# microsoft/GenerativeImage2Text

Measured on AMD Instinct MI355X. Metric: captions/sec whole-node (GIT_BASE 224px bs=64/GPU greedy len=20), higher is better.
Workload: dtype f16; 1 GPU; GIT_BASE 224px bs=64/GPU greedy max_len=20 frames=1; global_batch=64, parallelism=dp1, decode_steps_per_caption=19, seq_len_returned=20, hip_graph=True, contexts_in_flight=4, layernorm_folded=True, library=libgitmi_f16.so, encoder_chains=2, schedule=mixed

## Files before the change

generativeimage2text_amd/csrc/kernels_gemm10.hip:

```cpp
#include "gitmi_common.h"
#include "launchers.h"
#include <type_traits>

namespace gitmi {

namespace {

constexpr int BN = 256, BK = 64;
constexpr int HALF_BYTES = 128 * BK * 2;
constexpr int BUF_BYTES = 4 * HALF_BYTES;
constexpr int LDS_BYTES = 2 * BUF_BYTES;
constexpr int SLOT_A0 = 0, SLOT_A1 = HALF_BYTES, SLOT_B0 = 2 * HALF_BYTES, SLOT_B1 = 3 * HALF_BYTES;

typedef __attribute__((address_space(3))) void lds_void_t;

#define P8_BARRIER()                           \
    do {                                       \
        __builtin_amdgcn_sched_barrier(0);     \
        __builtin_amdgcn_s_barrier();          \
        asm volatile("" ::: "memory");         \
        __builtin_amdgcn_sched_barrier(0);     \
    } while (0)

__device__ __forceinline__ float add_unfused(float a, float b) {
// ... 25 lines not shown
#define P8_LDS_BARRIER()                                   \
    do {                                                   \
        asm volatile("s_waitcnt lgkmcnt(0)" ::: "memory"); \
        __builtin_amdgcn_s_barrier();                      \
        asm volatile("" ::: "memory");                     \
    } while (0)

template <typename T> __device__ __forceinline__ uint32_t pack2o(float lo, float hi) {
    if constexpr (std::is_same<T, f16_t>::value) return pack2h(lo, hi);
    else return pack2bf(lo, hi);
}
template <typename T> __device__ __forceinline__ void unpack2o(uint32_t u, float& lo, float& hi) {
    if constexpr (std::is_same<T, f16_t>::value) unpack2h(u, lo, hi);
    else unpack2op(u, lo, hi);
}

template <int N> __device__ __forceinline__ void wait_vm() {
    if constexpr (N == 8) asm volatile("s_waitcnt vmcnt(8)" ::: "memory");
    else if constexpr (N == 4) asm volatile("s_waitcnt vmcnt(4)" ::: "memory");
    else if constexpr (N == 2) asm volatile("s_waitcnt vmcnt(2)" ::: "memory");
    else if constexpr (N == 0) asm volatile("s_waitcnt vmcnt(0)" ::: "memory");
}

template <typename TOut, int ACT, int DBG = 0, int MH = 128, int EPI = 1, int MH1 = MH, int LNF = 0>
__global__ __launch_bounds__(512) void gemm_p8_kernel(GemmArgs g) {
    static_assert(LNF == 0 || sizeof(TOut) == 2, "LayerNorm folding: 16-bit outputs only");
    static_assert(MH % 32 == 0 && MH1 % 32 == 0 && MH1 <= MH && MH <= 128, "half tiles: multiples of 32 rows, second <= first");
    constexpr int BM = MH + MH1, MI = MH / 32, MI1 = MH1 / 32;
    __shared__ __attribute__((aligned(16))) unsigned char smem[LDS_BYTES];

    const int tid = threadIdx.x;
    const int lane = tid & 63;
    const int wave = __builtin_amdgcn_readfirstlane(tid >> 6);
    const int grp = wave >> 2, wc = wave & 3;
    const int l15 = lane & 15, lg = lane >> 4;
    uint64_t ts[8];
    auto stamp = [&](int i) {
        if constexpr ((DBG & 16) != 0) {
            __builtin_amdgcn_sched_barrier(0);
            ts[2 * i] = __builtin_amdgcn_s_memtime();
            ts[2 * i + 1] = __builtin_amdgcn_s_memrealtime();
            __builtin_amdgcn_sched_barrier(0);
        }
    };
    auto stamps_out = [&]() {
        if constexpr ((DBG & 16) != 0) {
            if (tid == 0) {
                uint64_t* o = reinterpret_cast<uint64_t*>(const_cast<float*>(g.res)) + (size_t)blockIdx.x * 8;
#pragma unroll
                for (int i = 0; i < 8; ++i) o[i] = ts[i];
            }
        }
// ... 97 lines not shown
        __builtin_amdgcn_sched_barrier(0);
        read_a(sb, H0);
        if constexpr (MODE <= 1) { issue(1, 1, t + 1); wait_vm<8>(); } else { wait_vm<2>(); }
        P8_BARRIER();
        mma(acc[0][0], wf0, H0);
        P8_BARRIER();
        read_w(sb, 1, wf1);
        if constexpr (MODE <= 1) { issue(0, 1, t + 1); wait_vm<8>(); } else { wait_vm<0>(); }
        P8_BARRIER();
        mma(acc[0][1], wf1, H0);
        P8_BARRIER();
        read_a(sb, H1);
        if constexpr (MODE == 0) { issue(0, 0, t + 2); wait_vm<8>(); }
        P8_BARRIER();
        mma(acc[1][1], wf1, H1);
        P8_BARRIER();
        if constexpr (MODE == 0) { issue(1, 0, t + 2); wait_vm<8>(); }
        else if constexpr (MODE == 1) { wait_vm<4>(); }
        P8_BARRIER();
        mma(acc[1][0], wf0, H1);
        P8_BARRIER();
    };

    float lmean[2][MI], lrstd[2][MI];
    unsigned char* const ln_lds = smem + BUF_BYTES + SLOT_A1;
    if constexpr (LNF == 1) {
        const int r = lane >> 1, qm = r >> 4, l = r & 15;
        const int MHq = qm ? MH1 : MH, MIq = qm ? MI1 : MI;
        const int ii = wc < MIq ? wc : MIq - 1;
        const int m = m0 + qm * MH + grp * (MHq / 2) + ii * 16 + l;
        const int mc = m < g.M ? m : g.M - 1;
        const char* src = reinterpret_cast<const char*>(g.ln_part) + (size_t)mc * 32 + (lane & 1) * 16;
        __builtin_amdgcn_global_load_lds((const void*)src, (lds_void_t*)(ln_lds + wave * 1024), 16, 0, 0);
    }
    auto ln_rows = [&]() {
        if constexpr (LNF == 1) {
#pragma unroll
            for (int qm = 0; qm < 2; ++qm) {
                const int MIq = qm ? MI1 : MI;
                const int ii = lg < MIq ? lg : MIq - 1;
                const unsigned char* pr = ln_lds + (grp * 4 + ii) * 1024 + (qm * 16 + l15) * 32;
                const f32x4_t p0 = *reinterpret_cast<const f32x4_t*>(pr);
                const f32x4_t p1 = *reinterpret_cast<const f32x4_t*>(pr + 16);
                const float sx = (p0[0] + p0[2]) + (p1[0] + p1[2]);
                const float sq = (p0[1] + p0[3]) + (p1[1] + p1[3]);
                const float mean = sx * g.ln_inv_d;
                const float rstd = rsqrtf(fmaxf(sq * g.ln_inv_d - mean * mean, 0.f) + g.ln_eps);
#pragma unroll
                for (int i = 0; i < MIq; ++i) {
                    lmean[qm][i] = __shfl(mean, i * 16 + l15, 64);
                    lrstd[qm][i] = __shfl(rstd, i * 16 + l15, 64);
                    asm volatile("" : "+v"(lmean[qm][i]), "+v"(lrstd[qm][i]));
                }
            }
            __builtin_amdgcn_sched_barrier(0);
        }
    };
    const int nk = g.K / BK;
    issue(0, 0, 0); issue(1, 0, 0); issue(1, 1, 0); issue(0, 1, 0); issue(0, 0, 1); issue(1, 0, 1);
    wait_vm<8>();
    P8_BARRIER();
    ln_rows();
#pragma unroll
    for (int a = 0; a < 2; ++a)
#pragma unroll
        for (int b = 0; b < 2; ++b)
#pragma unroll
            for (int j = 0; j < 2; ++j)
#pragma unroll
                for (int i = 0; i < MI; ++i) acc[a][b][j][i] = f32x4_t{0.f, 0.f, 0.f, 0.f};
    if (grp == 1) P8_BARRIER();
    stamp(1);
    for (int t = 0; t < nk - 2; ++t) ktile(std::integral_constant<int, 0>{}, t);
    ktile(std::integral_constant<int, 1>{}, nk - 2);
    ktile(std::integral_constant<int, 2>{}, nk - 1);
    if (grp == 0) P8_BARRIER();
// ... 19 lines not shown
#pragma unroll
                    for (int i = 0; i < MI; ++i) sum += acc[a][b][j][i][0] + acc[a][b][j][i][1] + acc[a][b][j][i][2] + acc[a][b][j][i][3];
        if (sum == 12345.678f) C[0] = (TOut)0;
        stamp(3);
        stamps_out();
        return;
    }
    f32x4_t bias4[2][2];
#pragma unroll
    for (int qn = 0; qn < 2; ++qn)
#pragma unroll
        for (int j = 0; j < 2; ++j)
            bias4[qn][j] = g.bias ? *reinterpret_cast<const f32x4_t*>(g.bias + n0 + qn * 128 + wc * 32 + j * 16 + lg * 4)
                                  : f32x4_t{0.f, 0.f, 0.f, 0.f};

    f32x4_t cs4[2][2];
    if constexpr (LNF == 1) {
#pragma unroll
        for (int qn = 0; qn < 2; ++qn)
#pragma unroll
            for (int j = 0; j < 2; ++j)
                cs4[qn][j] = *reinterpret_cast<const f32x4_t*>(g.ln_colsum + n0 + qn * 128 + wc * 32 + j * 16 + lg * 4);
    }
    auto ln_apply = [&](float a, int qm, int qn, int j, int i, int r) -> float {
        if constexpr (LNF == 1) return lrstd[qm][i] * fmaf(-lmean[qm][i], cs4[qn][j][r], a);
        else return a;
    };

    if constexpr (sizeof(TOut) == 4 && EPI == 1) {
        float* Cf = reinterpret_cast<float*>(g.C);
        const float* R = g.res;
        const int col0 = n0 + wc * 32 + lg * 4;
        const bool has_res = R != nullptr && !(DBG & 1);
#pragma unroll
        for (int qm = 0; qm < 2; ++qm) {
            const int MIq = qm ? MI1 : MI, MHq = qm ? MH1 : MH;
            f32x4_t rr[MI][2][2];
            if (has_res) {
#pragma unroll
                for (int i = 0; i < MIq; ++i) {
                    const int m = m0 + qm * MH + grp * (MHq / 2) + i * 16 + l15;
                    const int mc = m < g.M ? m : g.M - 1;
                    const float* rp = R + (size_t)mc * g.ldr + col0;
#pragma unroll
                    for (int qn = 0; qn < 2; ++qn)
#pragma unroll
                        for (int j = 0; j < 2; ++j)
                            rr[i][qn][j] = *reinterpret_cast<const f32x4_t*>(rp + qn * 128 + j * 16);
// ... 9 lines not shown
#pragma unroll
                    for (int j = 0; j < 2; ++j) {
                        f32x4_t v;
#pragma unroll
                        for (int r = 0; r < 4; ++r) v[r] = apply_act_t<ACT>(acc[qm][qn][j][i][r] + bias4[qn][j][r]);
                        if (has_res) {
#pragma unroll
                            for (int r = 0; r < 4; ++r) v[r] = add_unfused(v[r], rr[i][qn][j][r]);
                        }
                        if (ok) *reinterpret_cast<f32x4_t*>(cp + qn * 128 + j * 16) = v;
                    }
            }
        }
        return;
    }

    float rgm[8], rbt[8];
    if constexpr (LNF == 2) {
        if (g.res_part) {
            ld8(g.res_gamma + n0 + (tid & 31) * 8, rgm);
            ld8(g.res_beta + n0 + (tid & 31) * 8, rbt);
        }
    }
#pragma unroll
    for (int qm = 0; qm < 2; ++qm)
#pragma unroll
        for (int s = 0; s < 2 / NQN; ++s) {
            const int MIq = qm ? MI1 : MI, MHq = qm ? MH1 : MH;
#pragma unroll
            for (int u = 0; u < NQN; ++u) {
                const int qn = s * NQN + u;
#pragma unroll
                for (int j = 0; j < 2; ++j) {
                    const int nl = u * 128 + wc * 32 + j * 16 + lg * 4;
#pragma unroll
                    for (int i = 0; i < MIq; ++i) {
                        float v[4];
#pragma unroll
                        for (int r = 0; r < 4; ++r) v[r] = apply_act_t<ACT>(ln_apply(acc[qm][qn][j][i][r], qm, qn, j, i, r) + bias4[qn][j][r]);
                        TOut* p = ep + (grp * (MHq / 2) + i * 16 + l15) * EPS + nl;
                        if constexpr (sizeof(TOut) == 4) {
                            *reinterpret_cast<f32x4_t*>(p) = f32x4_t{v[0], v[1], v[2], v[3]};
                        } else {
                            uint2 t2;
                            t2.x = pack2o<TOut>(v[0], v[1]);
                            t2.y = pack2o<TOut>(v[2], v[3]);
                            *reinterpret_cast<uint2*>(p) = t2;
                        }
                    }
                }
            }
            P8_LDS_BARRIER();
#pragma unroll 4
            for (int q = 0; q < MHq * CPR / 512; ++q) {
                const int chunk = tid + q * 512;
                const int row = chunk / CPR, cc = chunk % CPR;
                const int m = m0 + qm * MH + row;
                const int n = n0 + s * WCOL + cc * EPC;
                if (m < g.M && !(DBG & 1)) {
                    if constexpr (sizeof(TOut) == 4) {
                        f32x4_t v = *reinterpret_cast<const f32x4_t*>(ep + row * EPS + cc * EPC);
                        if (g.res && !(DBG & 16)) {
// ... 69 lines not shown
                            q2 = __builtin_elementwise_fma(x, x, q2);
                        }
                        float sx = s2[0] + s2[1], sq = q2[0] + q2[1];
                        half_wave_sum2_hi(sx, sq);
                        if (ok && cc == 16 && !(DBG & 1)) g.part_out[(size_t)m * 4 + tile_n] = float2{sx, sq};
                    }
                    if (ok && !(DBG & 1)) {
                        TOut* cp = C + (size_t)m * g.ldc + n;
                        asm volatile("global_store_dwordx4 %0, %1, off sc1\n\ts_nop 1" ::"v"(cp), "v"(v) : "memory");
                    }
                }
            }
            P8_LDS_BARRIER();
        }
    if constexpr ((DBG & 16) != 0) {
        asm volatile("s_waitcnt vmcnt(0)" ::: "memory");
        stamp(3);
        stamps_out();
    }
}

}

template <typename TOut, int MH, int EPI = 1, int MH1 = MH, int LNF = 0>
static void launch_p8_t(const GemmArgs& g, hipStream_t s) {
    if constexpr (LNF == 2) {
        hipLaunchKernelGGL((gemm_p8_kernel<TOut, GITMI_ACT_NONE, 0, MH, EPI, MH1, LNF>), dim3(g.nwg), dim3(512), 0, s, g);
        return;
    } else {
    if (g.dbg && LNF == 0) {
        if constexpr (MH == 128 && MH1 == 128) {
            switch (g.dbg) {
                case 1: hipLaunchKernelGGL((gemm_p8_kernel<TOut, 0, 1>), dim3(g.nwg), dim3(512), 0, s, g); return;
                case 2: hipLaunchKernelGGL((gemm_p8_kernel<TOut, 0, 2>), dim3(g.nwg), dim3(512), 0, s, g); return;
                case 6: hipLaunchKernelGGL((gemm_p8_kernel<TOut, 0, 6>), dim3(g.nwg), dim3(512), 0, s, g); return;
                case 10: hipLaunchKernelGGL((gemm_p8_kernel<TOut, 0, 10>), dim3(g.nwg), dim3(512), 0, s, g); return;
#ifdef GITMI_PROBE
                case 16: hipLaunchKernelGGL((gemm_p8_kernel<TOut, 0, 16>), dim3(g.nwg), dim3(512), 0, s, g); return;
                case 17: hipLaunchKernelGGL((gemm_p8_kernel<TOut, 0, 17>), dim3(g.nwg), dim3(512), 0, s, g); return;
                case 18: hipLaunchKernelGGL((gemm_p8_kernel<TOut, 0, 18>), dim3(g.nwg), dim3(512), 0, s, g); return;
                case 22: hipLaunchKernelGGL((gemm_p8_kernel<TOut, 0, 22>), dim3(g.nwg), dim3(512), 0, s, g); return;
                case 26: hipLaunchKernelGGL((gemm_p8_kernel<TOut, 0, 26>), dim3(g.nwg), dim3(512), 0, s, g); return;
#endif
                default: break;
            }
        }
    }
    switch (g.act) {
        case GITMI_ACT_QUICKGELU:
            hipLaunchKernelGGL((gemm_p8_kernel<TOut, GITMI_ACT_QUICKGELU, 0, MH, EPI, MH1, LNF>), dim3(g.nwg), dim3(512), 0, s, g); break;
        case GITMI_ACT_GELU_ERF:
            hipLaunchKernelGGL((gemm_p8_kernel<TOut, GITMI_ACT_GELU_ERF, 0, MH, EPI, MH1, LNF>), dim3(g.nwg), dim3(512), 0, s, g); break;
        default:
            hipLaunchKernelGGL((gemm_p8_kernel<TOut, GITMI_ACT_NONE, 0, MH, EPI, MH1, LNF>), dim3(g.nwg), dim3(512), 0, s, g); break;
    }
    }
}

bool gemm_p8_supports(const GemmArgs& g) {
    return g.K % BK == 0 && g.K >= 2 * BK && g.N % BN == 0 &&
           (double)g.M * g.lda * 2.0 < 4.0e9 && (double)g.N * g.K * 2.0 < 4.0e9;
}

static int p8_xcd_count(const GemmArgs& g, int bm, int ng, int* max_nn_out) {
    const int tiles_m = (g.M + bm - 1) / bm, tiles_n = g.N / BN, mg = 8 / ng;
    int max_cnt = 0, max_nn = 0;
    for (int x = 0; x < 8; ++x) {
        const int gn = x % ng, gm = x / ng;
        const int nn = (gn + 1) * tiles_n / ng - gn * tiles_n / ng;
        const int tg = tiles_m * nn;
        const int cnt = (gm + 1) * tg / mg - gm * tg / mg;
        max_cnt = cnt > max_cnt ? cnt : max_cnt;
        max_nn = nn > max_nn ? nn : max_nn;
    }
    if (max_nn_out) *max_nn_out = max_nn;
    return max_cnt;
}
static int p8_plan(const GemmArgs& g, int bm, int* ng_out, int* max_cnt_out) {
    const int tiles_n = g.N / BN;
    int best_ng = 1, best_rounds = 1 << 30, best_cnt = 0, best_panels = 1 << 30;
    for (int ng = 1; ng <= 8 && ng <= tiles_n; ng *= 2) {
        int max_nn = 0;
        const int max_cnt = p8_xcd_count(g, bm, ng, &max_nn);
        const int rounds = (max_cnt + 31) / 32;
        const int panels = (32 + max_nn - 1) / max_nn + (max_nn < 32 ? max_nn : 32);
        if (rounds < best_rounds || (rounds == best_rounds && panels < best_panels)) {
            best_ng = ng; best_rounds = rounds; best_cnt = max_cnt; best_panels = panels;
        }
    }
    if (ng_out) *ng_out = best_ng;
    if (max_cnt_out) *max_cnt_out = best_cnt;
    return best_rounds;
}

int gemm_p8_cost(const GemmArgs& g, int bm) {
    const int rounds = p8_plan(g, bm, nullptr, nullptr);
    const int ktile = 1450 * (90 + 166 * bm / 256) / 256;
    return rounds * (1450 + (g.K / BK) * ktile + 4700 * bm / 256);
}

template <int MH, int MH1>
static void launch_p8_height(const GemmArgs& g, bool out_f32, bool staged, hipStream_t s) {
#ifdef GITMI_OPS_F16
    if (g.ln_part) { launch_p8_t<bf16_t, MH, 1, MH1, 1>(g, s); return; }
    if (g.part_out || g.res_part) { launch_p8_t<f16_t, MH, 1, MH1, 2>(g, s); return; }
#endif
    if (g.out_f16) launch_p8_t<f16_t, MH, 1, MH1>(g, s);
    else if (!out_f32) launch_p8_t<bf16_t, MH, 1, MH1>(g, s);
    else if (staged) launch_p8_t<float, MH, 0, MH1>(g, s);
    else launch_p8_t<float, MH, 1, MH1>(g, s);
}

hipError_t launch_gemm_p8(GemmArgs g, bool out_f32, hipStream_t s) {
    if (g.ln_part || g.part_out || g.res_part) {
#ifndef GITMI_OPS_F16
        return hipErrorInvalidValue;
#endif
        if (g.ln_part && (out_f32 || g.out_f16 || g.res || !g.ln_colsum || g.ln_nparts < 1 || g.part_out || g.res_part)) return hipErrorInvalidValue;
        if ((g.part_out || g.res_part) && (!g.out_f16 || out_f32 || g.act != 0 || g.N > 1024)) return hipErrorInvalidValue;
        if (g.res_part && (!g.res || !g.res_gamma || !g.res_beta || g.res_nparts < 1)) return hipErrorInvalidValue;
    }
    static const int heights[5] = {256, 224, 192, 160, 128};
    int bm = 256;
    if (!g.shared) {
        int best = gemm_p8_cost(g, 256);
        for (int h = 1; h < 5; ++h) {
            const int c = gemm_p8_cost(g, heights[h]);
            if (c < best) { best = c; bm = heights[h]; }
        }
    }
    if (g.dbg & 64) bm = 192;
    if (g.dbg & 128) bm = 256;
    if (g.dbg & 16384) bm = 160;
    if (g.dbg & 32768) bm = 224;
    if (g.dbg & 65536) bm = 128;
    g.dbg &= ~(64 | 128 | 16384 | 32768 | 65536);
    g.tiles_n = g.N / BN;
    int max_cnt = 0;
    p8_plan(g, bm, &g.ng, &max_cnt);
    if (g.dbg & (1024 | 2048 | 4096 | 8192)) {
        const int ng = (g.dbg & 1024) ? 1 : (g.dbg & 2048) ? 2 : (g.dbg & 4096) ? 4 : 8;
        g.dbg &= ~(1024 | 2048 | 4096 | 8192);
        if (ng <= g.tiles_n) { g.ng = ng; max_cnt = p8_xcd_count(g, bm, ng, nullptr); }
    }
    g.nwg = 8 * max_cnt;
    const bool staged = (g.dbg & 256) != 0;
    g.dbg &= ~256;
    switch (bm) {
        case 224: launch_p8_height<128, 96>(g, out_f32, staged, s); break;
        case 192: launch_p8_height<96, 96>(g, out_f32, staged, s); break;
        case 160: launch_p8_height<96, 64>(g, out_f32, staged, s); break;
        case 128: launch_p8_height<64, 64>(g, out_f32, staged, s); break;
        default: launch_p8_height<128, 128>(g, out_f32, staged, s); break;
    }
    return hipGetLastError();
}

}
```

generativeimage2text_amd/engine.py:

```python
from __future__ import annotations

import ctypes as C
import os
from typing import Dict, List, Mapping, Optional, Sequence, Tuple

import torch

_HERE = os.path.dirname(os.path.abspath(__file__))
LIB_PATH = os.path.join(_HERE, "libgitmi.so")
LIB_PATH_F16 = os.path.join(_HERE, "libgitmi_f16.so")
LIB_PATH_EXP = os.path.join(_HERE, "libgitmi_exp.so")

PREC_BF16, PREC_F32 = 0, 1
DTYPE_F32, DTYPE_BF16, DTYPE_F16 = 0, 1, 2
DTYPE_F16_STREAM = 3
SEARCH_AUTOREGRESSIVE, SEARCH_GENERATOR, SEARCH_TRIE = 0, 1, 2
SEARCH_SCORE = 3
SEARCH_ATTEND = 4
ACT_NONE, ACT_QUICKGELU, ACT_GELU_ERF = 0, 1, 2

EXPORTED_SYMBOLS = [
    "gitmi_abi_version", "gitmi_last_error", "gitmi_create", "gitmi_destroy", "gitmi_load_tensor",
    "gitmi_finalize_weights", "gitmi_encode_frames", "gitmi_prefill", "gitmi_step_logits",
    "gitmi_generate", "gitmi_search_begin", "gitmi_search_rows", "gitmi_search_advance",
    "gitmi_search_finish", "gitmi_profile_enable", "gitmi_profile_read", "gitmi_set_graph",
    "gitmi_op_gemm", "gitmi_op_layernorm", "gitmi_op_attention", "gitmi_op_dgemm", "gitmi_op_dgemm_res",
    "gitmi_op_vocab_topm", "gitmi_clone", "gitmi_op_attn_decode", "gitmi_preprocess_image",
    "gitmi_set_image_shape", "gitmi_preprocess_image_to", "gitmi_generate_prefixed", "gitmi_set_temporal_embedding", "gitmi_op_kv_repack", "gitmi_set_encode_after", "gitmi_op_sample_rows",
    "gitmi_search_done_count", "gitmi_set_trie", "gitmi_operand_dtype", "gitmi_set_shared_device", "gitmi_preprocess_batch",
    "gitmi_set_ln_fold", "gitmi_op_gemm_ln",
]
EXPERIMENT_SYMBOLS = [
    "gitmi_debug_import_stage", "gitmi_debug_head_from", "gitmi_debug_set_gemm_impl", "gitmi_debug_set_dgemm",
    "gitmi_debug_score_attn", "gitmi_debug_score_head", "gitmi_debug_attention_ragged", "gitmi_debug_attn_decode_ragged",
# ... 15 lines not shown
                ("max_steps", C.c_int32), ("length_penalty", C.c_double),
                ("do_sample", C.c_int32), ("top_k", C.c_int32), ("top_p", C.c_double), ("temperature", C.c_double),
                ("seed", C.c_uint64), ("repetition_penalty", C.c_double),
                ("num_keep_best", C.c_int32), ("reserved_", C.c_int32)]


class GitmiProfile(C.Structure):
    _fields_ = [("vit_ms", C.c_float), ("prefill_ms", C.c_float), ("decode_ms", C.c_float),
                ("total_ms", C.c_float), ("gemm_ms", C.c_float), ("gemm_launches", C.c_int32),
                ("gemm_flops", C.c_double), ("vit_gemm_ms", C.c_float), ("vit_gemm_launches", C.c_int32),
                ("vit_gemm_flops", C.c_double), ("decode_step_ms", C.c_float), ("decode_steps", C.c_int32),
                ("decode_step_bytes", C.c_double)]

    def as_dict(self) -> Dict[str, float]:
        return {n: getattr(self, n) for n, _ in self._fields_}


class GitmiError(RuntimeError):
    pass


_libs: Dict[str, C.CDLL] = {}
_experiment = False


def use_experiment_build(on: bool = True) -> None:
    global _experiment
    _experiment = bool(on)


def load_library(operands: str = "bf16") -> C.CDLL:
    if operands == "bf16" and _experiment:
        operands = "exp"
    if operands in _libs:
        return _libs[operands]
    path = {"bf16": LIB_PATH, "f16": LIB_PATH_F16, "exp": LIB_PATH_EXP}[operands]
    if not os.path.exists(path):
        raise GitmiError(
            f"{path} not found: build it with `python -c 'import __graft_entry__ as g; g.build()'` "
            f"or `make -C generativeimage2text_amd/csrc`.  There is no CPU fallback.")
    lib = C.CDLL(path)
    vp, i32, i64p, fp = C.c_void_p, C.c_int, C.POINTER(C.c_int64), C.c_void_p
    lib.gitmi_abi_version.restype = C.c_int
    lib.gitmi_last_error.restype = C.c_char_p
    lib.gitmi_create.argtypes = [C.POINTER(GitmiConfig), i32, C.POINTER(vp)]
    lib.gitmi_destroy.argtypes = [vp]
    lib.gitmi_destroy.restype = None
    lib.gitmi_load_tensor.argtypes = [vp, C.c_char_p, vp, i64p, i32, i32]
    lib.gitmi_finalize_weights.argtypes = [vp]
    lib.gitmi_encode_frames.argtypes = [vp, C.POINTER(vp), i32, i32, vp, vp]
    lib.gitmi_prefill.argtypes = [vp, vp]
    lib.gitmi_step_logits.argtypes = [vp, vp, i32, i32, vp, vp]
    lib.gitmi_generate.argtypes = [vp, C.POINTER(vp), i32, i32, vp, i32, C.POINTER(GitmiSearch), vp, vp, vp, vp]
    lib.gitmi_search_begin.argtypes = [vp, C.POINTER(GitmiSearch), i32, vp, i32, i32, vp]
    lib.gitmi_search_rows.argtypes = [vp, vp, C.POINTER(C.c_int), C.POINTER(C.c_int), vp]
    lib.gitmi_search_advance.argtypes = [vp, vp, vp]
    lib.gitmi_search_finish.argtypes = [vp, vp, vp, vp, vp]
    lib.gitmi_search_done_count.argtypes = [vp, C.POINTER(C.c_int), vp]
    lib.gitmi_set_trie.argtypes = [vp, i32, vp, vp, vp]
# ... 1 lines not shown
    lib.gitmi_profile_read.argtypes = [vp, C.POINTER(GitmiProfile)]
    lib.gitmi_set_graph.argtypes = [vp, i32]
    lib.gitmi_set_temporal_embedding.argtypes = [vp, i32]
    lib.gitmi_set_encode_after.argtypes = [vp, vp]
    lib.gitmi_set_shared_device.argtypes = [vp, i32]
    lib.gitmi_set_ln_fold.argtypes = [vp, i32]
    lib.gitmi_op_gemm.argtypes = [vp, vp, vp, vp, vp, i32, i32, i32, i32, i32, i32, i32, i32, vp]
    lib.gitmi_op_gemm_ln.argtypes = [vp, vp, vp, vp, vp, C.c_float, vp, vp, vp, vp, C.c_float, vp, vp, i32, i32, i32, i32, vp]
    lib.gitmi_op_layernorm.argtypes = [vp, vp, vp, C.c_float, vp, vp, i32, i32, i32, vp]
    lib.gitmi_op_attention.argtypes = [vp, vp, i32, i32, i32, i32, i32, vp]
    lib.gitmi_op_dgemm.argtypes = [vp, vp, vp, vp, vp, i32, C.c_float, vp, i32, i32, i32, i32, i32, i32, vp]
    lib.gitmi_op_dgemm_res.argtypes = [vp, vp, vp, vp, vp, i32, vp, vp, C.c_float, vp, vp, vp, i32, i32, i32, vp]
    lib.gitmi_op_vocab_topm.argtypes = [vp, vp, vp, vp, vp, i32, C.c_float, i32, i32, i32, i32, i32, vp, vp, vp, vp, vp, i32, vp]
    lib.gitmi_generate_prefixed.argtypes = [vp, C.POINTER(vp), i32, i32, vp, i32, C.POINTER(C.c_int32), C.POINTER(C.c_int32),
                                            i32, C.POINTER(GitmiSearch), vp, vp, vp, vp, vp]
    lib.gitmi_clone.argtypes = [vp, C.POINTER(vp)]
    lib.gitmi_preprocess_image.argtypes = [vp, i32, i32, i32, vp, C.c_size_t, vp, vp]
    lib.gitmi_preprocess_image_to.argtypes = [vp, i32, i32, i32, i32, vp, C.c_size_t, vp, vp]
    lib.gitmi_preprocess_batch.argtypes = [vp, C.c_size_t, i64p, i32, i32, vp, C.c_size_t, vp, vp]
    lib.gitmi_set_image_shape.argtypes = [vp, i32, i32, vp]
    lib.gitmi_op_attn_decode.argtypes = [vp, vp, vp, vp, vp, vp, vp, i32, i32, i32, i32, i32, i32, i32, i32, vp]
    lib.gitmi_op_kv_repack.argtypes = [vp, vp, vp, i32, i32, i32, vp]
    lib.gitmi_op_sample_rows.argtypes = [vp, i32, i32, C.c_float, i32, C.c_float, i32, C.c_uint64, i32, vp, vp, vp, vp]
    if operands == "exp":
        lib.gitmi_debug_import_stage.argtypes = [vp, vp, i32, vp]
        lib.gitmi_debug_head_from.argtypes = [vp, vp, i32, vp, vp]
        lib.gitmi_debug_set_gemm_impl.argtypes = [i32]
        lib.gitmi_debug_set_dgemm.argtypes = [i32]
        lib.gitmi_debug_dgemm_form.argtypes = [vp, i32, vp, vp, vp, vp, i32, C.c_float, vp, i32, i32, vp, vp, i32, vp, vp, C.c_float,
                                               vp, vp, vp, i32, i32, i32, i32, i32, i32, vp]
        lib.gitmi_debug_score_attn.argtypes = [vp, vp, vp, vp, i32, i32, i32, i32, i32, vp]
        lib.gitmi_debug_score_head.argtypes = [vp, vp, vp, vp, i32, i32, i32, i32, vp, vp]
        lib.gitmi_debug_score_attn_map.argtypes = [vp, vp, vp, vp, vp, i32, i32, i32, i32, i32, vp]
        lib.gitmi_debug_attention_ragged.argtypes = [vp, vp, vp, i32, i32, i32, i32, i32, vp]
        lib.gitmi_debug_attn_decode_ragged.argtypes = [vp, vp, vp, vp, vp, vp, vp, vp, i32, i32, i32, i32, i32, i32, i32, vp]
        lib.gitmi_debug_attn_decode_form.argtypes = [vp, vp, vp, vp, vp, vp, vp, vp, vp, i32, i32, i32, i32, i32, i32, i32, i32, i32,
                                                     i32, i32, i32, vp]
        lib.gitmi_debug_vocab_topm_rules.argtypes = [vp, vp, vp, vp, vp, i32, C.c_float, i32, i32, i32, i32, i32, vp, i32, i32, vp, i32,
                                                     i32, C.c_float, vp, vp, vp, vp, i32, vp]
        lib.gitmi_debug_search_begin_prefixed.argtypes = [vp, C.POINTER(GitmiSearch), i32, vp, i32, vp, i32, vp]
        lib.gitmi_debug_search_advance_lists.argtypes = [vp, vp, vp, vp, i32, i32, i32, vp]
        lib.gitmi_debug_read_hidden.argtypes = [vp, i32, vp, vp, C.POINTER(C.c_int), C.POINTER(C.c_int), vp]
        lib.gitmi_debug_im2col.argtypes = [vp, vp, i32, i32, i32, i32, i32, i32, i32, vp]
        lib.gitmi_debug_pos_resize.argtypes = [vp, vp, i32, i32, i32, i32, vp]
        lib.gitmi_debug_vit_assemble.argtypes = [vp, vp, vp, vp, vp, C.c_float, vp, i32, i32, i32, i32, vp, vp]
        lib.gitmi_debug_ragged_front.argtypes = [i32, vp, vp, vp, vp, vp, i32, vp, vp, vp, i32, vp, vp, C.c_float, vp, i32, vp, i32, i32,
                                                 C.c_longlong, i32, i32, i32, i32, vp]
        lib.gitmi_debug_zero_pad_rows.argtypes = [vp, i32, i32, vp, i32, i32, vp]
        lib.gitmi_debug_layernorm_map.argtypes = [vp, i32, vp, vp, C.c_float, vp, vp, i32, vp, i32, i32, i32, i32, i32, vp]
    for name in EXPORTED_SYMBOLS + (EXPERIMENT_SYMBOLS if operands == "exp" else []):
        if name not in ("gitmi_last_error", "gitmi_destroy"):
            getattr(lib, name).restype = C.c_int
    if lib.gitmi_abi_version() != 10:
        raise GitmiError("libgitmi.so ABI version mismatch")
    lib.gitmi_operand_dtype.restype = C.c_int
    if lib.gitmi_operand_dtype() != {"bf16": DTYPE_BF16, "f16": DTYPE_F16, "exp": DTYPE_BF16}[operands]:
        raise GitmiError(f"{path} was not built for {operands} operands")
    _libs[operands] = lib
    return lib


def _experiment_only(lib, name: str):
    try:
        return getattr(lib, name)
    except AttributeError:
        raise GitmiError(f"{name} is exported by the measurement build only (libgitmi_exp.so): call "
                         f"generativeimage2text_amd.engine.use_experiment_build() before creating the engine") from None


def _ck(rc: int, lib=None) -> None:
    if rc != 0:
        libs = [lib] if lib is not None else list(_libs.values())
        msgs = [m for m in ((l.gitmi_last_error() or b"").decode("utf-8", "replace") for l in libs) if m]
        raise GitmiError(" | ".join(msgs) or "gitmi call failed")


def _stream() -> int:
    return int(torch.cuda.current_stream().cuda_stream)

# ... 494 lines not shown

    def set_shared_device(self, on: bool = True) -> None:
        self._ck(self.lib.gitmi_set_shared_device(self._h, 1 if on else 0))

    def set_encode_after(self, other: Optional["Engine"]) -> None:
        self._ck(self.lib.gitmi_set_encode_after(self._h, other._h if other is not None else None))

    def set_temporal_embedding(self, on: bool) -> None:
        self._ck(self.lib.gitmi_set_temporal_embedding(self._h, 1 if on else 0))
        if bool(on) != self._temb:
            self._temb = bool(on)
            self._drop_resident()

    def set_ln_fold(self, on: bool) -> None:
        self._ck(self.lib.gitmi_set_ln_fold(self._h, 1 if on else 0))
        if bool(on) != self._ln_fold:
            self._ln_fold = bool(on)
            self._drop_resident()

    def set_graph(self, on: bool) -> None:
        self._ck(self.lib.gitmi_set_graph(self._h, 1 if on else 0))


def op_gemm(A: torch.Tensor, W: torch.Tensor, bias: Optional[torch.Tensor] = None,
            residual: Optional[torch.Tensor] = None, act: int = ACT_NONE,
            out_dtype: torch.dtype = torch.float32, stream_rows: bool = False) -> torch.Tensor:
    assert A.is_cuda and W.is_cuda and A.dtype == W.dtype and A.is_contiguous() and W.is_contiguous()
    M, K = A.shape
    N = W.shape[0]
    if stream_rows:
        if A.dtype == torch.float32:
            raise GitmiError("op_gemm: fp16 stream rows need 16-bit operands")
        if residual is not None and (residual.dtype != torch.float16 or residual.shape != (M, N) or not residual.is_contiguous()):
            raise GitmiError("op_gemm: the stream form's residual is contiguous fp16 [M, N] rows")
        lib, out_code, out_dtype = _op_library(A.dtype), DTYPE_F16_STREAM, torch.float16
    else:
        if residual is not None and residual.dtype != torch.float32:
            raise GitmiError("op_gemm: the residual is fp32 (fp16 rows: stream_rows=True)")
        lib = _op_library(A.dtype, out_dtype, fp32_ok=True)
        out_code = {torch.float32: DTYPE_F32, torch.bfloat16: DTYPE_BF16, torch.float16: DTYPE_F16}[out_dtype]
    out = torch.empty(M, N, device=A.device, dtype=out_dtype)
    _ck(lib.gitmi_op_gemm(A.data_ptr(), W.data_ptr(), _ptr(bias), _ptr(residual), out.data_ptr(), M, N, K, K, N,
                          _torch_dtype_code(A), out_code, act, _stream()), lib)
    return out


def op_gemm_ln(A: torch.Tensor, W: torch.Tensor, bias: Optional[torch.Tensor], *, colsum: Optional[torch.Tensor] = None,
               ln_part: Optional[torch.Tensor] = None, ln_eps: float = 1e-5, residual: Optional[torch.Tensor] = None,
               res_part: Optional[torch.Tensor] = None, res_gamma: Optional[torch.Tensor] = None,
               res_beta: Optional[torch.Tensor] = None, res_eps: float = 1e-12, want_part: bool = False, act: int = ACT_NONE):
    lib = load_library("f16")
    assert A.dtype == torch.float16 and W.dtype == torch.float16 and A.is_contiguous() and W.is_contiguous()
    M, K = A.shape
    N = W.shape[0]
    out = torch.empty(M, N, device=A.device, dtype=torch.float16)
    part = torch.zeros(M, 4, 2, device=A.device, dtype=torch.float32) if want_part else None
    _ck(lib.gitmi_op_gemm_ln(A.data_ptr(), W.data_ptr(), _ptr(bias), _ptr(colsum), _ptr(ln_part), ln_eps, _ptr(residual),
                             _ptr(res_part), _ptr(res_gamma), _ptr(res_beta), res_eps, out.data_ptr(), _ptr(part), M, N, K, act,
                             _stream()), lib)
    return (out, part) if want_part else out


def op_layernorm(x: torch.Tensor, gamma: torch.Tensor, beta: torch.Tensor, eps: float,
                 out_dtype: torch.dtype = torch.float32) -> torch.Tensor:
    lib = _op_library(out_dtype, fp32_ok=True)
    rows, D = x.shape
    out = torch.empty(rows, D, device=x.device, dtype=out_dtype)
    _ck(lib.gitmi_op_layernorm(x.data_ptr(), gamma.data_ptr(), beta.data_ptr(), eps, out.data_ptr(), None, rows, D,
                               _torch_dtype_code(out), _stream()), lib)
    return out


def op_attention(qkv: torch.Tensor, B: int, N: int, H: int, impl: int) -> torch.Tensor:
    lib = _op_library(qkv.dtype, fp32_ok=True)
    assert qkv.is_cuda and qkv.is_contiguous() and qkv.shape == (B * N, 3 * H * 64)
    out = torch.empty(B * N, H * 64, device=qkv.device, dtype=qkv.dtype)
    _ck(lib.gitmi_op_attention(qkv.data_ptr(), out.data_ptr(), B, N, H, _torch_dtype_code(qkv), impl, _stream()), lib)
    return out

# ... 122 lines not shown
    lib, _, ops, shape, outs, result, keep = _vocab_head_call(A, W, bias, mtop, cols_per_wg, colsum, stats, want_logits, packed, rows, V)
    _ck(lib.gitmi_op_vocab_topm(*ops, eps, *shape, _ptr(suppress_tok), *outs, int(max_wgs), _stream()), lib)
    return result


def op_vocab_topm_rules(A: torch.Tensor, W: torch.Tensor, bias: torch.Tensor, mtop: int, ids: Optional[torch.Tensor],
                        cur_len: int, plen: Optional[torch.Tensor], beams: int = 1, suppress_kind: int = 0,
                        rep_penalty: float = 0.0, cols_per_wg: int = 128, colsum: Optional[torch.Tensor] = None,
                        stats: Optional[torch.Tensor] = None, eps: float = 1e-12, want_logits: bool = False, packed: bool = False,
                        rows: Optional[int] = None, V: Optional[int] = None, max_wgs: int = 0):
    lib, M, ops, shape, outs, result, keep = _vocab_head_call(A, W, bias, mtop, cols_per_wg, colsum, stats, want_logits, packed, rows, V)
    if ids is not None:
        ids = ids.to(device=A.device, dtype=torch.int32).contiguous()
        plen = plen.to(device=A.device, dtype=torch.int32).contiguous()
        if ids.dim() != 2 or ids.shape[0] != M or plen.numel() * beams != M:
            raise ValueError(f"ids {tuple(ids.shape)} / plen {tuple(plen.shape)} do not describe {M} rows of {beams} beams")
    _ck(_experiment_only(lib, "gitmi_debug_vocab_topm_rules")(
        *ops, eps, *shape, _ptr(ids), 0 if ids is None else int(ids.shape[1]), int(cur_len), _ptr(plen), int(beams),
        int(suppress_kind), float(rep_penalty), *outs, int(max_wgs), _stream()), lib)
    return result


def set_gemm_impl(impl: int) -> None:
    lib = load_library()
    _ck(_experiment_only(lib, "gitmi_debug_set_gemm_impl")(int(impl)), lib)


def op_attn_decode(qkv, img_k, img_v, txt_k, txt_v, kv_src, B, H, N_img, T_max, pos, beams, dbg=0):
    lib = _op_library(qkv.dtype, img_k.dtype, img_v.dtype, txt_k.dtype, txt_v.dtype, fp32_ok=True)
    R, d = B * beams, H * 64
    out = torch.empty(R, d, device=qkv.device, dtype=qkv.dtype)
    if qkv.dtype != torch.float32 and img_k.dim() == 4:
        img_k, img_v = kv_repack(img_k, img_v)
    _ck(lib.gitmi_op_attn_decode(qkv.data_ptr(), img_k.data_ptr(), img_v.data_ptr(), txt_k.data_ptr(), txt_v.data_ptr(),
                                 kv_src.data_ptr(), out.data_ptr(), B, H, N_img, T_max, pos, beams, _torch_dtype_code(qkv),
                                 dbg, _stream()), lib)
    return out


def op_attention_ragged(qkv: torch.Tensor, ntok, B: int, N: int, H: int, impl: int) -> torch.Tensor:
    lib = load_library()
    nt = torch.as_tensor(ntok, dtype=torch.int32).to(qkv.device)
    out = torch.empty(B * N, H * 64, device=qkv.device, dtype=qkv.dtype)
    _ck(_experiment_only(lib, "gitmi_debug_attention_ragged")(qkv.data_ptr(), out.data_ptr(), nt.data_ptr(), B, N, H,
                                                              _torch_dtype_code(qkv), impl, _stream()), lib)
    return out


# ... 187 lines not shown
```

Before: 11300 captions/s.

## Stage 16-bit GEMM epilogue through swizzled LDS for coalesced row stores

Adds a new default epilogue path for 16-bit outputs in the p8 GEMM. Accumulators are written into a swizzled LDS slab, then each thread copies full 16-byte row segments to global memory, with residual, LayerNorm-residual and partial-stat handling done on the coalesced rows. LayerNorm mean/rstd values are parked in a small LDS region instead of being held in per-lane registers via shuffles, which reduces register pressure. The old path stays reachable through an experiment debug flag, and the Python side gains optional preallocated out/part buffers and an f16 experiment library.

```diff
diff --git a/generativeimage2text_amd/csrc/kernels_gemm10.hip b/generativeimage2text_amd/csrc/kernels_gemm10.hip
--- a/generativeimage2text_amd/csrc/kernels_gemm10.hip
+++ b/generativeimage2text_amd/csrc/kernels_gemm10.hip
@@ -71,12 +71,13 @@
     else if constexpr (N == 0) asm volatile("s_waitcnt vmcnt(0)" ::: "memory");
 }
 
-template <typename TOut, int ACT, int DBG = 0, int MH = 128, int EPI = 1, int MH1 = MH, int LNF = 0>
+template <typename TOut, int ACT, int DBG = 0, int MH = 128, int EPI = 1, int MH1 = MH, int LNF = 0, int EP16 = 1>
 __global__ __launch_bounds__(512) void gemm_p8_kernel(GemmArgs g) {
     static_assert(LNF == 0 || sizeof(TOut) == 2, "LayerNorm folding: 16-bit outputs only");
     static_assert(MH % 32 == 0 && MH1 % 32 == 0 && MH1 <= MH && MH <= 128, "half tiles: multiples of 32 rows, second <= first");
     constexpr int BM = MH + MH1, MI = MH / 32, MI1 = MH1 / 32;
-    __shared__ __attribute__((aligned(16))) unsigned char smem[LDS_BYTES];
+    constexpr int PARK_BYTES = LNF == 1 ? 256 * 8 : 0;
+    __shared__ __attribute__((aligned(16))) unsigned char smem[LDS_BYTES + PARK_BYTES];
 
     const int tid = threadIdx.x;
     const int lane = tid & 63;
@@ -220,7 +221,7 @@
         P8_BARRIER();
     };
 
-    float lmean[2][MI], lrstd[2][MI];
+    float2* const park = reinterpret_cast<float2*>(smem + LDS_BYTES);
     unsigned char* const ln_lds = smem + BUF_BYTES + SLOT_A1;
     if constexpr (LNF == 1) {
         const int r = lane >> 1, qm = r >> 4, l = r & 15;
@@ -244,12 +245,7 @@
                 const float sq = (p0[1] + p0[3]) + (p1[1] + p1[3]);
                 const float mean = sx * g.ln_inv_d;
                 const float rstd = rsqrtf(fmaxf(sq * g.ln_inv_d - mean * mean, 0.f) + g.ln_eps);
-#pragma unroll
-                for (int i = 0; i < MIq; ++i) {
-                    lmean[qm][i] = __shfl(mean, i * 16 + l15, 64);
-                    lrstd[qm][i] = __shfl(rstd, i * 16 + l15, 64);
-                    asm volatile("" : "+v"(lmean[qm][i]), "+v"(lrstd[qm][i]));
-                }
+                if (wc == 0 && lg < MIq) park[qm * MH + grp * ((qm ? MH1 : MH) / 2) + lg * 16 + l15] = float2{mean, rstd};
             }
             __builtin_amdgcn_sched_barrier(0);
         }
@@ -315,8 +311,12 @@
             for (int j = 0; j < 2; ++j)
                 cs4[qn][j] = *reinterpret_cast<const f32x4_t*>(g.ln_colsum + n0 + qn * 128 + wc * 32 + j * 16 + lg * 4);
     }
-    auto ln_apply = [&](float a, int qm, int qn, int j, int i, int r) -> float {
-        if constexpr (LNF == 1) return lrstd[qm][i] * fmaf(-lmean[qm][i], cs4[qn][j][r], a);
+    auto ln_row = [&](int qm, int i, int l15) -> float2 {
+        if constexpr (LNF == 1) return park[qm * MH + grp * ((qm ? MH1 : MH) / 2) + i * 16 + l15];
+        else return float2{0.f, 0.f};
+    };
+    auto ln_apply = [&](float a, float2 mr, int qn, int j, int r) -> float {
+        if constexpr (LNF == 1) return mr.y * fmaf(-mr.x, cs4[qn][j][r], a);
         else return a;
     };
 
@@ -372,6 +372,174 @@
             ld8(g.res_beta + n0 + (tid & 31) * 8, rbt);
         }
     }
+    if constexpr (sizeof(TOut) == 2 && EP16 != 0) {
+        constexpr int NQ = BM / 16;
+        constexpr bool RES16 = LNF == 2 || std::is_same<TOut, f16_t>::value;
+        int te = tid;
+        asm volatile("" : "+v"(te));
+        const int l15 = te & 15, lg = (te >> 4) & 3, lane = te & 63;
+        const int xw = ((l15 & 7) << 1) | (l15 >> 3);
+        int wcol[2];
+#pragma unroll
+        for (int j = 0; j < 2; ++j) wcol[j] = ((wc * 8 + j * 4 + lg) ^ xw) * 8;
+        auto stage = [&](auto qm_c) __attribute__((always_inline)) {
+            constexpr int qm = decltype(qm_c)::value;
+            constexpr int MIq = qm ? MI1 : MI, MHq = qm ? MH1 : MH;
+#pragma unroll
+            for (int i = 0; i < MIq; ++i) {
+                const float2 mr = ln_row(qm, i, l15);
+                unsigned char* prow = smem + (qm * MH + grp * (MHq / 2) + i * 16 + l15) * 512;
+#pragma unroll
+                for (int qn = 0; qn < 2; ++qn)
+#pragma unroll
+                    for (int j = 0; j < 2; ++j) {
+                        float v[4];
+#pragma unroll
+                        for (int r = 0; r < 4; ++r) v[r] = apply_act_t<ACT>(ln_apply(acc[qm][qn][j][i][r], mr, qn, j, r) + bias4[qn][j][r]);
+                        uint2 t2;
+                        t2.x = pack2o<TOut>(v[0], v[1]);
+                        t2.y = pack2o<TOut>(v[2], v[3]);
+                        *reinterpret_cast<uint2*>(prow + qn * 256 + wcol[j]) = t2;
+                    }
+            }
+        };
+        const int rrow = te >> 5, cc = te & 31;
+        const int n = n0 + cc * EPC;
+        const unsigned char* rd = smem + rrow * 512 + ((cc ^ (rrow & 7)) * 16);
+        auto copy_out = [&](auto has_res_c) __attribute__((always_inline)) {
+            constexpr bool HAS_RES = decltype(has_res_c)::value;
+            stage(H0);
+            u32x4_t rr[RES16 ? NQ : 1];
+            f32x4_t rf[RES16 ? 1 : NQ][2];
+            float pmean = 0.f, prstd = 0.f;
+            f32x4_t pp0 = {0.f, 0.f, 0.f, 0.f}, pp1 = pp0;
+            if constexpr (HAS_RES) {
+                if constexpr (LNF == 2) {
+                    if (g.res_part) {
+                        const int kk = (lane & 15) < NQ ? (lane & 15) : NQ - 1;
+                        const int m = m0 + kk * 16 + rrow;
+                        const int mc = m < g.M ? m : g.M - 1;
+                        const f32x4_t* pp = reinterpret_cast<const f32x4_t*>(g.res_part + (size_t)mc * 4);
+                        pp0 = pp[0]; pp1 = pp[1];
+                    }
+                }
+#pragma unroll
+                for (int k = 0; k < NQ; ++k) {
+                    const int m = m0 + k * 16 + rrow;
+                    const int mc = m < g.M ? m : g.M - 1;
+                    if constexpr (RES16) {
+                        rr[k] = *reinterpret_cast<const u32x4_t*>(reinterpret_cast<const f16_t*>(g.res) + (size_t)mc * g.ldr + n);
+                    } else {
+                        const float* rp = g.res + (size_t)mc * g.ldr + n;
+                        rf[k][0] = *reinterpret_cast<const f32x4_t*>(rp);
+                        rf[k][1] = *reinterpret_cast<const f32x4_t*>(rp + 4);
+                    }
+                }
+            }
+            P8_LDS_BARRIER();
+            if constexpr (HAS_RES) {
+                if constexpr (LNF == 2) {
+                    if (g.res_part) {
+                        const f32x4_t p0 = pp0, p1 = pp1;
+                        const float mean = ((p0[0] + p0[2]) + (p1[0] + p1[2])) * g.res_inv_d;
+                        const float rstd = rsqrtf(fmaxf(((p0[1] + p0[3]) + (p1[1] + p1[3])) * g.res_inv_d - mean * mean, 0.f) + g.res_eps);
+                        pmean = mean; prstd = rstd;
+                    }
+                }
+#pragma unroll
+                for (int k = 0; k < NQ; ++k) {
+                    if constexpr (RES16) asm volatile("" : "+v"(rr[k]));
+                    else asm volatile("" : "+v"(rf[k][0]), "+v"(rf[k][1]));
+                }
+            }
+            auto copy_rows = [&](auto k0_c, auto k1_c) __attribute__((always_inline)) {
+#pragma unroll
+            for (int k = decltype(k0_c)::value; k < decltype(k1_c)::value; ++k) {
+                const int m = m0 + k * 16 + rrow;
+                const bool ok = m < g.M && !(DBG & 1);
+                u32x4_t v = *reinterpret_cast<const u32x4_t*>(rd + k * 16 * 512);
+                if (grp) v = u32x4_t{v[2], v[3], v[0], v[1]};
+                if constexpr (LNF == 2) {
+                    float f[8];
+#pragma unroll
+                    for (int e = 0; e < 4; ++e) unpack2h(v[e], f[2 * e], f[2 * e + 1]);
+                    if constexpr (HAS_RES) {
+                        float rs[8];
+#pragma unroll
+                        for (int e = 0; e < 4; ++e) unpack2h(rr[k][e], rs[2 * e], rs[2 * e + 1]);
+                        if (g.res_part) {
+                            const float mean = __shfl(pmean, (lane & 32) + k, 64);
+                            const float rstd = __shfl(prstd, (lane & 32) + k, 64);
+#pragma unroll
+                            for (int e = 0; e < 8; ++e) rs[e] = fmaf((rs[e] - mean) * rstd, rgm[e], rbt[e]);
+                        }
+#pragma unroll
+                        for (int e = 0; e < 8; ++e) f[e] += rs[e];
+#pragma unroll
+                        for (int e = 0; e < 4; ++e) v[e] = pack2h(f[2 * e], f[2 * e + 1]);
+                    }
+                    if (g.part_out) {
+                        typedef __attribute__((ext_vector_type(2))) float f32x2_t;
+                        f32x2_t s2 = {0.f, 0.f}, q2 = {0.f, 0.f};
+#pragma unroll
+                        for (int e = 0; e < 4; ++e) {
+                            float x0, x1;
+                            unpack2h(v[e], x0, x1);
+                            const f32x2_t x = {x0, x1};
+                            s2 += x;
+                            q2 = __builtin_elementwise_fma(x, x, q2);
+                        }
+                        float sx = s2[0] + s2[1], sq = q2[0] + q2[1];
+                        half_wave_sum2_hi(sx, sq);
+                        if (ok && cc == 16) g.part_out[(size_t)m * 4 + tile_n] = float2{sx, sq};
+                    }
+                    if (ok) {
+                        TOut* cp = C + (size_t)m * g.ldc + n;
+                        asm volatile("global_store_dwordx4 %0, %1, off sc1\n\ts_nop 1" ::"v"(cp), "v"(v) : "memory");
+                    }
+                } else if (ok) {
+                    if constexpr (HAS_RES) {
+                        float f[8], rs[8];
+#pragma unroll
+                        for (int e = 0; e < 4; ++e) unpack2o<TOut>(v[e], f[2 * e], f[2 * e + 1]);
+                        if constexpr (RES16) {
+#pragma unroll
+                            for (int e = 0; e < 4; ++e) unpack2h(rr[k][e], rs[2 * e], rs[2 * e + 1]);
+                        } else {
+#pragma unroll
+                            for (int e = 0; e < 4; ++e) { rs[e] = rf[k][0][e]; rs[4 + e] = rf[k][1][e]; }
+                        }
+#pragma unroll
+                        for (int e = 0; e < 8; ++e) f[e] += rs[e];
+#pragma unroll
+                        for (int e = 0; e < 4; ++e) v[e] = pack2o<TOut>(f[2 * e], f[2 * e + 1]);
+                    }
+                    TOut* cp = C + (size_t)m * g.ldc + n;
+                    if (g.dbg & 512)
+                        *reinterpret_cast<u32x4_t*>(cp) = v;
+                    else
+                        asm volatile("global_store_dwordx4 %0, %1, off sc1\n\ts_nop 1" ::"v"(cp), "v"(v) : "memory");
+                }
+            }
+            };
+            constexpr std::integral_constant<int, 0> K0{};
+            constexpr std::integral_constant<int, MH / 16> KH{};
+            constexpr std::integral_constant<int, NQ> KN{};
+            copy_rows(K0, KH);
+            stage(H1);
+            P8_LDS_BARRIER();
+            copy_rows(KH, KN);
+        };
+        if (g.res != nullptr && !(DBG & 17)) copy_out(std::true_type{});
+        else copy_out(std::false_type{});
+        if constexpr ((DBG & 16) != 0) {
+            asm volatile("s_waitcnt vmcnt(0)" ::: "memory");
+            stamp(3);
+            stamps_out();
+        }
+        return;
+    }
+
 #pragma unroll
     for (int qm = 0; qm < 2; ++qm)
 #pragma unroll
@@ -386,8 +554,9 @@
 #pragma unroll
                     for (int i = 0; i < MIq; ++i) {
                         float v[4];
-#pragma unroll
-                        for (int r = 0; r < 4; ++r) v[r] = apply_act_t<ACT>(ln_apply(acc[qm][qn][j][i][r], qm, qn, j, i, r) + bias4[qn][j][r]);
+                        const float2 mr = ln_row(qm, i, l15);
+#pragma unroll
+                        for (int r = 0; r < 4; ++r) v[r] = apply_act_t<ACT>(ln_apply(acc[qm][qn][j][i][r], mr, qn, j, r) + bias4[qn][j][r]);
                         TOut* p = ep + (grp * (MHq / 2) + i * 16 + l15) * EPS + nl;
                         if constexpr (sizeof(TOut) == 4) {
                             *reinterpret_cast<f32x4_t*>(p) = f32x4_t{v[0], v[1], v[2], v[3]};
@@ -503,10 +672,10 @@
 
 }
 
-template <typename TOut, int MH, int EPI = 1, int MH1 = MH, int LNF = 0>
+template <typename TOut, int MH, int EPI = 1, int MH1 = MH, int LNF = 0, int EP16 = 1>
 static void launch_p8_t(const GemmArgs& g, hipStream_t s) {
     if constexpr (LNF == 2) {
-        hipLaunchKernelGGL((gemm_p8_kernel<TOut, GITMI_ACT_NONE, 0, MH, EPI, MH1, LNF>), dim3(g.nwg), dim3(512), 0, s, g);
+        hipLaunchKernelGGL((gemm_p8_kernel<TOut, GITMI_ACT_NONE, 0, MH, EPI, MH1, LNF, EP16>), dim3(g.nwg), dim3(512), 0, s, g);
         return;
     } else {
     if (g.dbg && LNF == 0) {
@@ -529,11 +698,11 @@
     }
     switch (g.act) {
         case GITMI_ACT_QUICKGELU:
-            hipLaunchKernelGGL((gemm_p8_kernel<TOut, GITMI_ACT_QUICKGELU, 0, MH, EPI, MH1, LNF>), dim3(g.nwg), dim3(512), 0, s, g); break;
+            hipLaunchKernelGGL((gemm_p8_kernel<TOut, GITMI_ACT_QUICKGELU, 0, MH, EPI, MH1, LNF, EP16>), dim3(g.nwg), dim3(512), 0, s, g); break;
         case GITMI_ACT_GELU_ERF:
-            hipLaunchKernelGGL((gemm_p8_kernel<TOut, GITMI_ACT_GELU_ERF, 0, MH, EPI, MH1, LNF>), dim3(g.nwg), dim3(512), 0, s, g); break;
+            hipLaunchKernelGGL((gemm_p8_kernel<TOut, GITMI_ACT_GELU_ERF, 0, MH, EPI, MH1, LNF, EP16>), dim3(g.nwg), dim3(512), 0, s, g); break;
         default:
-            hipLaunchKernelGGL((gemm_p8_kernel<TOut, GITMI_ACT_NONE, 0, MH, EPI, MH1, LNF>), dim3(g.nwg), dim3(512), 0, s, g); break;
+            hipLaunchKernelGGL((gemm_p8_kernel<TOut, GITMI_ACT_NONE, 0, MH, EPI, MH1, LNF, EP16>), dim3(g.nwg), dim3(512), 0, s, g); break;
     }
     }
 }
@@ -580,14 +749,25 @@
     return rounds * (1450 + (g.K / BK) * ktile + 4700 * bm / 256);
 }
 
-template <int MH, int MH1>
+template <int MH, int MH1, bool SLAB = false>
 static void launch_p8_height(const GemmArgs& g, bool out_f32, bool staged, hipStream_t s) {
+#ifdef GITMI_EXPERIMENT
+    if constexpr (!SLAB) {
+        if ((g.dbg & 32) && !out_f32) {
+            GemmArgs h = g;
+            h.dbg &= ~32;
+            launch_p8_height<MH, MH1, true>(h, out_f32, staged, s);
+            return;
+        }
+    }
+#endif
+    constexpr int EP16 = SLAB ? 0 : 1;
 #ifdef GITMI_OPS_F16
-    if (g.ln_part) { launch_p8_t<bf16_t, MH, 1, MH1, 1>(g, s); return; }
-    if (g.part_out || g.res_part) { launch_p8_t<f16_t, MH, 1, MH1, 2>(g, s); return; }
+    if (g.ln_part) { launch_p8_t<bf16_t, MH, 1, MH1, 1, EP16>(g, s); return; }
+    if (g.part_out || g.res_part) { launch_p8_t<f16_t, MH, 1, MH1, 2, EP16>(g, s); return; }
 #endif
-    if (g.out_f16) launch_p8_t<f16_t, MH, 1, MH1>(g, s);
-    else if (!out_f32) launch_p8_t<bf16_t, MH, 1, MH1>(g, s);
+    if (g.out_f16) launch_p8_t<f16_t, MH, 1, MH1, 0, EP16>(g, s);
+    else if (!out_f32) launch_p8_t<bf16_t, MH, 1, MH1, 0, EP16>(g, s);
     else if (staged) launch_p8_t<float, MH, 0, MH1>(g, s);
     else launch_p8_t<float, MH, 1, MH1>(g, s);
 }
@@ -627,6 +807,9 @@
     g.nwg = 8 * max_cnt;
     const bool staged = (g.dbg & 256) != 0;
     g.dbg &= ~256;
+#ifndef GITMI_EXPERIMENT
+    g.dbg &= ~32;
+#endif
     switch (bm) {
         case 224: launch_p8_height<128, 96>(g, out_f32, staged, s); break;
         case 192: launch_p8_height<96, 96>(g, out_f32, staged, s); break;
diff --git a/generativeimage2text_amd/engine.py b/generativeimage2text_amd/engine.py
--- a/generativeimage2text_amd/engine.py
+++ b/generativeimage2text_amd/engine.py
@@ -10,6 +10,7 @@
 LIB_PATH = os.path.join(_HERE, "libgitmi.so")
 LIB_PATH_F16 = os.path.join(_HERE, "libgitmi_f16.so")
 LIB_PATH_EXP = os.path.join(_HERE, "libgitmi_exp.so")
+LIB_PATH_F16_EXP = os.path.join(_HERE, "libgitmi_f16_exp.so")
 
 PREC_BF16, PREC_F32 = 0, 1
 DTYPE_F32, DTYPE_BF16, DTYPE_F16 = 0, 1, 2
@@ -71,19 +72,23 @@
 
 _libs: Dict[str, C.CDLL] = {}
 _experiment = False
-
-
-def use_experiment_build(on: bool = True) -> None:
-    global _experiment
+_experiment_f16 = False
+
+
+def use_experiment_build(on: bool = True, f16: bool = False) -> None:
+    global _experiment, _experiment_f16
     _experiment = bool(on)
+    _experiment_f16 = bool(on) and bool(f16)
 
 
 def load_library(operands: str = "bf16") -> C.CDLL:
     if operands == "bf16" and _experiment:
         operands = "exp"
+    if operands == "f16" and _experiment_f16:
+        operands = "f16_exp"
     if operands in _libs:
         return _libs[operands]
-    path = {"bf16": LIB_PATH, "f16": LIB_PATH_F16, "exp": LIB_PATH_EXP}[operands]
+    path = {"bf16": LIB_PATH, "f16": LIB_PATH_F16, "exp": LIB_PATH_EXP, "f16_exp": LIB_PATH_F16_EXP}[operands]
     if not os.path.exists(path):
         raise GitmiError(
             f"{path} not found: build it with `python -c 'import __graft_entry__ as g; g.build()'` "
@@ -131,7 +136,7 @@
     lib.gitmi_op_attn_decode.argtypes = [vp, vp, vp, vp, vp, vp, vp, i32, i32, i32, i32, i32, i32, i32, i32, vp]
     lib.gitmi_op_kv_repack.argtypes = [vp, vp, vp, i32, i32, i32, vp]
     lib.gitmi_op_sample_rows.argtypes = [vp, i32, i32, C.c_float, i32, C.c_float, i32, C.c_uint64, i32, vp, vp, vp, vp]
-    if operands == "exp":
+    if operands in ("exp", "f16_exp"):
         lib.gitmi_debug_import_stage.argtypes = [vp, vp, i32, vp]
         lib.gitmi_debug_head_from.argtypes = [vp, vp, i32, vp, vp]
         lib.gitmi_debug_set_gemm_impl.argtypes = [i32]
@@ -157,13 +162,13 @@
                                                  C.c_longlong, i32, i32, i32, i32, vp]
         lib.gitmi_debug_zero_pad_rows.argtypes = [vp, i32, i32, vp, i32, i32, vp]
         lib.gitmi_debug_layernorm_map.argtypes = [vp, i32, vp, vp, C.c_float, vp, vp, i32, vp, i32, i32, i32, i32, i32, vp]
-    for name in EXPORTED_SYMBOLS + (EXPERIMENT_SYMBOLS if operands == "exp" else []):
+    for name in EXPORTED_SYMBOLS + (EXPERIMENT_SYMBOLS if operands in ("exp", "f16_exp") else []):
         if name not in ("gitmi_last_error", "gitmi_destroy"):
             getattr(lib, name).restype = C.c_int
     if lib.gitmi_abi_version() != 10:
         raise GitmiError("libgitmi.so ABI version mismatch")
     lib.gitmi_operand_dtype.restype = C.c_int
-    if lib.gitmi_operand_dtype() != {"bf16": DTYPE_BF16, "f16": DTYPE_F16, "exp": DTYPE_BF16}[operands]:
+    if lib.gitmi_operand_dtype() != {"bf16": DTYPE_BF16, "f16": DTYPE_F16, "exp": DTYPE_BF16, "f16_exp": DTYPE_F16}[operands]:
         raise GitmiError(f"{path} was not built for {operands} operands")
     _libs[operands] = lib
     return lib
@@ -704,9 +709,17 @@
         self._ck(self.lib.gitmi_set_graph(self._h, 1 if on else 0))
 
 
+def _op_out(out: Optional[torch.Tensor], M: int, N: int, device, dtype: torch.dtype) -> torch.Tensor:
+    if out is None:
+        return torch.empty(M, N, device=device, dtype=dtype)
+    if out.shape != (M, N) or out.dtype != dtype or not out.is_contiguous() or out.device != device:
+        raise GitmiError(f"out must be a contiguous {dtype} [{M}, {N}] tensor on the operands' device")
+    return out
+
+
 def op_gemm(A: torch.Tensor, W: torch.Tensor, bias: Optional[torch.Tensor] = None,
             residual: Optional[torch.Tensor] = None, act: int = ACT_NONE,
-            out_dtype: torch.dtype = torch.float32, stream_rows: bool = False) -> torch.Tensor:
+            out_dtype: torch.dtype = torch.float32, stream_rows: bool = False, out: Optional[torch.Tensor] = None) -> torch.Tensor:
     assert A.is_cuda and W.is_cuda and A.dtype == W.dtype and A.is_contiguous() and W.is_contiguous()
     M, K = A.shape
     N = W.shape[0]
@@ -721,7 +734,7 @@
             raise GitmiError("op_gemm: the residual is fp32 (fp16 rows: stream_rows=True)")
         lib = _op_library(A.dtype, out_dtype, fp32_ok=True)
         out_code = {torch.float32: DTYPE_F32, torch.bfloat16: DTYPE_BF16, torch.float16: DTYPE_F16}[out_dtype]
-    out = torch.empty(M, N, device=A.device, dtype=out_dtype)
+    out = _op_out(out, M, N, A.device, out_dtype)
     _ck(lib.gitmi_op_gemm(A.data_ptr(), W.data_ptr(), _ptr(bias), _ptr(residual), out.data_ptr(), M, N, K, K, N,
                           _torch_dtype_code(A), out_code, act, _stream()), lib)
     return out
@@ -730,13 +743,18 @@
 def op_gemm_ln(A: torch.Tensor, W: torch.Tensor, bias: Optional[torch.Tensor], *, colsum: Optional[torch.Tensor] = None,
                ln_part: Optional[torch.Tensor] = None, ln_eps: float = 1e-5, residual: Optional[torch.Tensor] = None,
                res_part: Optional[torch.Tensor] = None, res_gamma: Optional[torch.Tensor] = None,
-               res_beta: Optional[torch.Tensor] = None, res_eps: float = 1e-12, want_part: bool = False, act: int = ACT_NONE):
+               res_beta: Optional[torch.Tensor] = None, res_eps: float = 1e-12, want_part: bool = False, act: int = ACT_NONE,
+               out: Optional[torch.Tensor] = None, part: Optional[torch.Tensor] = None):
     lib = load_library("f16")
     assert A.dtype == torch.float16 and W.dtype == torch.float16 and A.is_contiguous() and W.is_contiguous()
     M, K = A.shape
     N = W.shape[0]
-    out = torch.empty(M, N, device=A.device, dtype=torch.float16)
-    part = torch.zeros(M, 4, 2, device=A.device, dtype=torch.float32) if want_part else None
+    out = _op_out(out, M, N, A.device, torch.float16)
+    if want_part and part is not None:
+        if part.shape != (M, 4, 2) or part.dtype != torch.float32 or not part.is_contiguous() or part.device != A.device:
+            raise GitmiError("op_gemm_ln: part must be a contiguous float32 [M, 4, 2] tensor on the operands' device")
+    else:
+        part = torch.zeros(M, 4, 2, device=A.device, dtype=torch.float32) if want_part else None
     _ck(lib.gitmi_op_gemm_ln(A.data_ptr(), W.data_ptr(), _ptr(bias), _ptr(colsum), _ptr(ln_part), ln_eps, _ptr(residual),
                              _ptr(res_part), _ptr(res_gamma), _ptr(res_beta), res_eps, out.data_ptr(), _ptr(part), M, N, K, act,
                              _stream()), lib)
@@ -905,8 +923,8 @@
 
 
 def set_gemm_impl(impl: int) -> None:
-    lib = load_library()
-    _ck(_experiment_only(lib, "gitmi_debug_set_gemm_impl")(int(impl)), lib)
+    for lib in [load_library()] + ([load_library("f16")] if _experiment_f16 else []):
+        _ck(_experiment_only(lib, "gitmi_debug_set_gemm_impl")(int(impl)), lib)
 
 
 def op_attn_decode(qkv, img_k, img_v, txt_k, txt_v, kv_src, B, H, N_img, T_max, pos, beams, dbg=0):
```

Measured after the change: 11430 captions/s, median of 6. 1.01x the previous value.
